# hcherkaoui/pybold

Measured on AMD Instinct MI355X. Metric: voxel-iterations/sec, higher is better.
Workload: dtype f16x2-split operands (22 bit), f32 accumulate, f64 iterate

## Files before the change

### include/pybold_hip.h

```cpp
#ifndef PYBOLD_HIP_H
#define PYBOLD_HIP_H

#include <stdint.h>

#ifdef __cplusplus
extern "C" {
#endif

#define PB_OK 0
#define PB_ERR_INVALID (-1)
#define PB_ERR_HIP (-2)

#define PB_FLAG_FORCE_GENERIC 1u
#define PB_FLAG_FORCE_FAST 2u
#define PB_FLAG_NO_PAIR 4u
#define PB_FLAG_FORCE_PAIR 8u
#define PB_FLAG_FORCE_WIDE 16u
#define PB_FLAG_DIRECT_FIR 64u
#define PB_FLAG_ONE_STREAM 128u
#define PB_FLAG_COLD_START 256u
#define PB_FLAG_NO_CERT 512u
#define PB_FLAG_CERT_NO_RESOLVE 2048u
#define PB_FLAG_FORCE_MFMA 16384u
#define PB_FLAG_NO_RHO_GUARD 32768u
// ... 18 lines not shown

int pb_fista_has_fast_path(int N, int K);

int pb_fista_which_kernel(int N, int K, int P, int with_cost_trace, int stop_mode, int wind);

int pb_fista_plan(int N, int K, int P, int stop_mode, int wind, int* n_main, int* main_form,
                  int* tail_form);
int pb_fista_plan_ex(int N, int K, int P, int stop_mode, int wind, unsigned flags, int* n_main,
                     int* main_form, int* tail_form);

int pb_fista_solve(const float* y_dev, int64_t ldy, int y_rep,
                   double* w_dev, int64_t ldw, int P, int N,
                   const double* taps_host, const double* taps_dev, int K,
                   double step, double lbda, const double* lbda_dev,
                   const double* betas_dev, int n_iter,
                   float* J_dev, int64_t ldj,
                   int stop_mode, double tol, int wind, int32_t* n_done_dev,
                   unsigned flags, void* stream);

int64_t pb_fista_work_len(int P, int y_rep);
#define PB_CAND_COUNT 10
int pb_fista_list_plan(int kind, int n, int n_max, int has_pair, int has_wide, int one_stream, int has_mfma2,
                       int beside_chunks, int32_t* ranges, int32_t* bounds);
int pb_fista_solve_ex(const float* y_dev, int64_t ldy, int y_rep,
                      double* w_dev, int64_t ldw, int P, int N,
                      const double* taps_host, const double* taps_dev, int K,
                      double step, double lbda, const double* lbda_dev,
                      const double* betas_dev, int n_iter,
                      float* J_dev, int64_t ldj,
                      int stop_mode, double tol, int wind, int32_t* n_done_dev,
                      unsigned flags, void* stream,
                      const double* lmax_dev, double dense_ratio, int32_t* work_dev, int64_t work_len);

#define PB_PATH_DENSE_RATIO 0.19
#define PB_PATH_DENSE_RATIO_LONG 0.22
#define PB_PATH_DENSE_RATIO_LONGER 0.26
int64_t pb_fista_path_work_len(int P);
int pb_fista_solve_path(const float* y_dev, int64_t ldy, int y_rep, double* w_dev, int64_t ldw, int P, int N,
                        const double* taps_host, const double* taps_dev, int K, double step,
                        const double* lbda_dev, const double* lmax_dev, double dense_ratio,
                        const double* betas_dev, int n_iter, int32_t* n_done_dev, int32_t* work_dev,
                        int64_t work_len, unsigned flags, void* stream);

int pb_fista_outputs(const double* w_dev, int64_t ldw, int P, int N,
                     const double* taps_dev, int K,
                     double* z_dev, int64_t ldz, double* x_dev, int64_t ldx,
// ... 138 lines not shown
```

### pybold_amd/_lib.py

```python
import ctypes
import os

_HERE = os.path.dirname(os.path.abspath(__file__))
LIB_PATH = os.environ.get("PYBOLD_HIP_LIB") or os.path.join(_HERE, "libpybold_hip.so")

PB_FLAG_FORCE_GENERIC = 1
PB_FLAG_FORCE_FAST = 2
PB_FLAG_NO_PAIR = 4
PB_FLAG_FORCE_PAIR = 8
PB_FLAG_FORCE_WIDE = 16
PB_FLAG_ONE_LAUNCH = 32
PB_FLAG_DIRECT_FIR = 64
PB_FLAG_ONE_STREAM = 128
PB_FLAG_COLD_START = 256
PB_FLAG_NO_CERT = 512
PB_FLAG_FORCE_CERT = 1024
PB_FLAG_CERT_NO_RESOLVE = 2048
PB_FLAG_NO_PARTITION = 4096
PB_FLAG_NO_MFMA = 8192
PB_FLAG_FORCE_MFMA = 16384
PB_FLAG_NO_RHO_GUARD = 32768
PB_FLAG_FORCE_MFMA2 = 65536
PB_FLAG_ONLY_DENSE = 131072
PB_FLAG_ONLY_SPARSE = 262144
# ... 7 lines not shown
_c_i64 = ctypes.c_int64
_c_dbl = ctypes.c_double
_ptr = ctypes.c_void_p

SIGNATURES = {
    "pb_version": (_c_int, []),
    "pb_init": (_c_int, []),
    "pb_last_error": (ctypes.c_char_p, []),
    "pb_fista_has_fast_path": (_c_int, [_c_int, _c_int]),
    "pb_fista_which_kernel": (_c_int, [_c_int, _c_int, _c_int, _c_int, _c_int, _c_int]),
    "pb_fista_plan": (_c_int, [_c_int, _c_int, _c_int, _c_int, _c_int, _ptr, _ptr, _ptr]),
    "pb_fista_plan_ex": (_c_int, [_c_int, _c_int, _c_int, _c_int, _c_int, ctypes.c_uint, _ptr, _ptr, _ptr]),
    "pb_fista_solve": (_c_int, [
        _ptr, _c_i64, _c_int,
        _ptr, _c_i64, _c_int, _c_int,
        _ptr, _ptr, _c_int,
        _c_dbl, _c_dbl, _ptr,
        _ptr, _c_int,
        _ptr, _c_i64,
        _c_int, _c_dbl, _c_int, _ptr,
        ctypes.c_uint, _ptr]),
    "pb_fista_work_len": (_c_i64, [_c_int, _c_int]),
    "pb_fista_list_plan": (_c_int, [_c_int, _c_int, _c_int, _c_int, _c_int, _c_int, _c_int, _c_int, _ptr, _ptr]),
    "pb_fista_solve_ex": (_c_int, [
        _ptr, _c_i64, _c_int,
        _ptr, _c_i64, _c_int, _c_int,
        _ptr, _ptr, _c_int,
        _c_dbl, _c_dbl, _ptr,
        _ptr, _c_int,
        _ptr, _c_i64,
        _c_int, _c_dbl, _c_int, _ptr,
        ctypes.c_uint, _ptr,
        _ptr, _c_dbl, _ptr, _c_i64]),
    "pb_fista_solve_backtrack_d": (_c_int, [
        _ptr, _c_i64, _c_int, _ptr, _c_i64, _c_int, _c_int,
        _ptr, _c_int, _c_dbl, _c_dbl, _c_int,
        _c_dbl, _ptr, _ptr, _c_int,
        _ptr, _ptr, _ptr, ctypes.c_uint, _ptr]),
    "pb_fista_path_work_len": (_c_i64, [_c_int]),
    "pb_fista_solve_path": (_c_int, [
        _ptr, _c_i64, _c_int,
        _ptr, _c_i64, _c_int, _c_int,
        _ptr, _ptr, _c_int,
        _c_dbl, _ptr, _ptr, _c_dbl,
        _ptr, _c_int,
        _ptr, _ptr, _c_i64,
# ... 133 lines not shown
```

### pybold_amd/csrc/capi.hip

```cpp
#include "../../include/pybold_hip.h"

#include <cstdarg>
#include <cstdlib>
#include <cstdio>
#include <cmath>
#include <cstring>
#include <map>
#include <mutex>

#include "fista_fast.h"
#include "generic.h"
#include "launch_fast.h"
#include "fista_pair.h"
#include "fista_pair_ffa.h"
#include "fista_exact.h"
#include "fista_exact_split.h"
#include "fista_auto.h"
#include "fista_exact_pp.h"
#include "blind.h"
#include "fista_mfma.h"
#include "fista_mfma2.h"
#include "fista_mfma4.h"
#include "path.h"
#include "dispatch.h"
// ... 35 lines not shown
  const int64_t rounds = ((int64_t)V + AUTO_SPLIT_RESIDENT_WGS - 1) / AUTO_SPLIT_RESIDENT_WGS;
  const int64_t per = (int64_t)(nb_sub_iter > 0 ? nb_sub_iter : 1) * (rounds > 0 ? rounds : 1);
  const int64_t c = AUTO_SPLIT_LAUNCH_ITERS / per;
  return (int)(c < 1 ? 1 : c);
}

constexpr int MAD_DAUB_NMAX = 8192;
template <typename TY>
int mad_daub_impl(const TY* y_dev, int64_t ldy, int V, int N, double c, double* sigma_dev, void* stream, const char* name) {
  if (V < 0 || ldy < N) return fail(PB_ERR_INVALID, "%s: bad size", name);
  if (N < 5 || N > MAD_DAUB_NMAX) return fail(PB_ERR_INVALID, "%s: N=%d outside 5..%d scans", name, N, MAD_DAUB_NMAX);
  if (!(c > 0.0)) return fail(PB_ERR_INVALID, "%s: c must be positive", name);
  if (V == 0) return PB_OK;
  if (!y_dev || !sigma_dev) return fail(PB_ERR_INVALID, "%s: NULL pointer", name);
  int n2 = 1;
  while (n2 < (N + 5) / 2) n2 <<= 1;
  hipLaunchKernelGGL((pb::mad_daub_kernel<TY>), dim3(V), dim3(pb::GEN_THREADS), (size_t)n2 * sizeof(double), (hipStream_t)stream,
                     y_dev, ldy, N, c, n2, sigma_dev);
  return check_launch(name);
}
struct SideStream {
  hipStream_t stream = nullptr;
  hipEvent_t fork = nullptr, join = nullptr;
  bool ok = false;
};
std::mutex g_side_mutex;

SideStream* side_stream_locked() {
  static std::map<int, SideStream> per_dev;
  int dev = 0;
  if (hipGetDevice(&dev) != hipSuccess) return nullptr;
  SideStream& ss = per_dev[dev];
  if (!ss.ok && ss.stream == nullptr) {
    int least = 0, greatest = 0;
    if (hipDeviceGetStreamPriorityRange(&least, &greatest) != hipSuccess) { least = greatest = 0; (void)hipGetLastError(); }
    if (hipStreamCreateWithPriority(&ss.stream, hipStreamNonBlocking, greatest) == hipSuccess &&
        hipEventCreateWithFlags(&ss.fork, hipEventDisableTiming) == hipSuccess &&
        hipEventCreateWithFlags(&ss.join, hipEventDisableTiming) == hipSuccess)
      ss.ok = true;
    else
      (void)hipGetLastError();
  }
  return ss.ok ? &ss : nullptr;
}

bool stream_is_capturing(hipStream_t st) {
  hipStreamCaptureStatus cs = hipStreamCaptureStatusNone;
  if (hipStreamIsCapturing(st, &cs) != hipSuccess) {
    (void)hipGetLastError();
    return true;
  }
  return cs != hipStreamCaptureStatusNone;
}
struct WorkLayout { int64_t ranges, lmax, total; };
WorkLayout work_layout(int P, int V) {
  const int64_t nblk = ((int64_t)P + pb::PATH_PER_BLOCK - 1) / pb::PATH_PER_BLOCK;
  WorkLayout w;
  w.ranges = ((int64_t)P + 2 + 2 * nblk + 8 + 1) & ~(int64_t)1;
  w.lmax = w.ranges + 3 * 2 * pb::CAND_COUNT + 4;
  w.total = w.lmax + 2 * (int64_t)V + 8;
  return w;
}
int32_t* own_workspace(void* stream, int64_t need, int64_t* len) {
  static std::mutex mu;
  static std::map<std::pair<int, void*>, std::pair<int32_t*, int64_t>> cache;
  int dev = 0;
  if (hipGetDevice(&dev) != hipSuccess) { (void)hipGetLastError(); return nullptr; }
  std::lock_guard<std::mutex> lock(mu);
  auto& e = cache[std::make_pair(dev, stream)];
  if (e.second < need) {
    int32_t* fresh = nullptr;
    const int64_t want = need + need / 4;
    if (hipMalloc((void**)&fresh, (size_t)want * sizeof(int32_t)) != hipSuccess) { (void)hipGetLastError(); return nullptr; }
    e.first = fresh;
    e.second = want;
  }
  *len = e.second;
  return e.first;
}

template <int KIND>
int launch_op(const double* x, int64_t ldx, double* out, int64_t ldo, int V, int n_src, int n_dst,
              const double* taps, int K, void* stream, const char* name) {
// ... 187 lines not shown
template <class LF>
int launch(const LF& lf, int form, const pb::FistaArgs& b, hipStream_t st, bool exact_rule = false) {
  static const char* const kernel[] = {"fista_generic_kernel", "fista_fast_kernel", "fista_pair_ffa_kernel", "fista_fast_kernel(wide)",
                                       "fista_mfma_kernel", "fista_mfma2_kernel / fista_mfma4_kernel"};
  if (lf(form, b, st, exact_rule) != 0) return fail(PB_ERR_INVALID, "%s: the kernel of form %d rejected its launch", lf.name, form);
  return check_launch(kernel[form]);
}

struct Side {
  std::unique_lock<std::mutex> lock{g_side_mutex, std::defer_lock};
  SideStream* ss = nullptr;
  bool forked = false;
  void take() {
    lock.lock();
    ss = side_stream_locked();
  }
  int fork(hipStream_t user, const char* name) {
    if (forked) return PB_OK;
    if (hipEventRecord(ss->fork, user) != hipSuccess || hipStreamWaitEvent(ss->stream, ss->fork, 0) != hipSuccess)
      return fail(PB_ERR_HIP, "%s: fork to the side stream failed", name);
    forked = true;
    return PB_OK;
  }
  int join(hipStream_t user, const char* name) {
    if (!forked) return PB_OK;
    forked = false;
    if (hipEventRecord(ss->join, ss->stream) != hipSuccess || hipStreamWaitEvent(user, ss->join, 0) != hipSuccess)
      return fail(PB_ERR_HIP, "%s: join of the side stream failed", name);
    return PB_OK;
  }
};

template <class LF>
int run_passes(const pb::FistaArgs& a, int base, int main_form, int rest_form, bool resolve, const LF& lf, hipStream_t st) {
  pb::FistaArgs b = a;
  if (base > 0) {
    b.P = base;
    const int rc = launch(lf, main_form, b, st);
    if (rc != PB_OK) return rc;
  }
  if (base < a.P) {
    b = a;
    b.p0 = base;
    const int rc = launch(lf, rest_form, b, st);
    if (rc != PB_OK) return rc;
  }
// ... 64 lines not shown
    s.dense.pass_mult = 2;
    s.dense.rem_num16 = MFMA4_MIN_R_NUM;
  }
  s.dense.backup_form = s.sparse.backup_form = s.flagged.backup_form = r.backup_wide ? FORM_WIDE : FORM_FAST1;
  s.sparse.min_pair = SPLIT_MIN_P;
  return s;
}
bool list_has_form(const Route& r, int form, int list) {
  const bool lng = r.path == PATH_PART_LONG;
  if (form == FORM_MFMA) return list <= 1 && r.mfma != nullptr;
  if (form == FORM_MFMA2) return list <= 1 && (lng || r.has_mfma2);
  if (list == 1) return false;
  if (form == FORM_PAIR) return list != 3 && r.has_pair;
  if (form == FORM_WIDE) return lng ? r.backup_wide : r.has_wide;
  return !lng || !r.backup_wide;
}
int cand_bound(const Route& r, int c, int P) {
  if (r.path == PATH_PART_SHORT) return pb::cand_max_slots(c, P, wave_slots());
  return (c == pb::CAND_MFMA2 || c == pb::CAND_PAIR0 || c == pb::CAND_FAST0 || c == pb::CAND_WIDE) ? P : 0;
}

template <class LF>
int solve_list(const Route& r, const pb::FistaArgs& a, const LF& lf, hipStream_t user, Side& side, const int32_t* work_dev,
               const int32_t* ranges, int list, bool exact_rule) {
  pb::FistaArgs b = a;
  b.perm = work_dev;
  b.n_dense = work_dev + a.P;
  b.perm_side = list == 3 ? 3 : 1;
  int rc = PB_OK;
  for (int c = 0; c < pb::CAND_COUNT && rc == PB_OK; ++c) {
    const int form = pb::cand_form(c);
    if (!list_has_form(r, form, list) || (pb::cand_side(c) && !side.ss)) continue;
    if ((c == pb::CAND_PAIR1 || c == pb::CAND_FAST1) && !side.ss) continue;
    b.grid_slots = cand_bound(r, c, a.P);
    if (b.grid_slots <= 0) continue;
    if (c >= pb::CAND_FIRST_AFTER_FORK && side.ss) rc = side.fork(user, lf.name);
    if (rc != PB_OK) break;
    b.range = ranges + 2 * c;
    rc = launch(lf, form, b, (pb::cand_side(c) && side.ss) ? side.ss->stream : user, exact_rule);
  }
  const int rj = side.join(user, lf.name);
  return rj != PB_OK ? rj : rc;
}

void launch_lmax_pass(const pb::FistaArgs& a, int V_series, const double* taps_host, double* lm, double gamma_f64, double gamma_vec,
                      hipStream_t st) {
  const int N = a.N, K = a.K;
  pb::LmaxTaps lt;
  double run = 0.0, csum = 0.0;
  for (int k = 0; k < pb::LMAX_KT; ++k) lt.h[k] = k < K ? (float)taps_host[k] : 0.0f;
  for (int t = 0; t < N; ++t) { if (t < K) run += taps_host[t]; csum += std::fabs(run); }
  const double unit = csum / std::sqrt((double)N);
  const float f64_bound = gamma_f64 > 0.0 ? (float)(gamma_f64 * unit) : 0.0f, vec_bound = gamma_vec > 0.0 ? (float)(gamma_vec * unit) : 0.0f;
  const dim3 grid((unsigned)((V_series + 3) / 4)), block(256);
  if (N <= 320) hipLaunchKernelGGL((pb::lmax_wave_kernel<5>), grid, block, 4 * (64 * 5 + pb::LMAX_KT) * sizeof(float), st, a.y, a.ldy, V_series, N, lt, K, lm, f64_bound, vec_bound);
  else if (N <= 640) hipLaunchKernelGGL((pb::lmax_wave_kernel<10>), grid, block, 4 * (64 * 10 + pb::LMAX_KT) * sizeof(float), st, a.y, a.ldy, V_series, N, lt, K, lm, f64_bound, vec_bound);
  else hipLaunchKernelGGL((pb::lmax_wave_kernel<21>), grid, block, 4 * (64 * 21 + pb::LMAX_KT) * sizeof(float), st, a.y, a.ldy, V_series, N, lt, K, lm, f64_bound, vec_bound);
}

int launch_partition(const pb::ClassPred& cp, int P, int32_t* work_dev, const pb::PlanSpec& front, const pb::PlanSpec& back,
                     int32_t* rg_front, int32_t* rg_back, int32_t* rg_ill, const char* what, hipStream_t st) {
  const int nblk = (P + pb::PATH_PER_BLOCK - 1) / pb::PATH_PER_BLOCK;
  hipLaunchKernelGGL(pb::path_count_kernel, dim3(nblk), dim3(pb::PATH_THREADS), 0, st, cp, P, work_dev);
  hipLaunchKernelGGL(pb::path_scan_kernel, dim3(1), dim3(pb::PATH_THREADS), 0, st, P, nblk, work_dev, front, back, rg_front, rg_back, rg_ill);
  hipLaunchKernelGGL(pb::path_scatter_kernel, dim3(nblk), dim3(pb::PATH_THREADS), 0, st, cp, P, work_dev);
  return check_launch(what);
}

void launch_generic(const pb::FistaArgs& a, const double* taps_dev, int K, int wind, bool with_j, bool f64, int grid, hipStream_t st) {
  void (*const kernel)(pb::FistaArgs, const double*, int, int) =
      !f64 ? (with_j ? pb::fista_generic_kernel<true> : pb::fista_generic_kernel<false>)
           : (with_j ? pb::fista_generic_kernel<true, true> : pb::fista_generic_kernel<false, true>);
  hipLaunchKernelGGL(kernel, dim3(grid), dim3(pb::GEN_THREADS), (size_t)gen_lds_doubles(a.N, K, a.stop_mode, wind) * sizeof(double), st,
                     a, taps_dev, K, wind);
}

template <class LF>
int run_partition(const Route& r, const pb::FistaArgs& a, const LF& lf, hipStream_t user, const double* taps_host,
                  const double* taps_dev, unsigned flags, double dense_ratio, int32_t* work_dev) {
  const int P = a.P, N = a.N, K = a.K, V_series = (P + a.y_rep - 1) / a.y_rep;
  const bool one_stream = r.path == PATH_PART_LONG || (flags & PB_FLAG_ONE_STREAM) != 0 || stream_is_capturing(user);
  const PartitionSpecs sp = partition_specs(r, N, one_stream);
  const WorkLayout wl = work_layout(P, V_series);
  const ExactEntry* ill_exact = pick_exact_any(N, K, a.stop_mode, a.wind, nullptr);
  const bool ill_generic = !ill_exact && taps_dev && gen_lds_doubles(N, K, a.stop_mode, a.wind) <= LDS_DOUBLES_MAX;
  const bool guard = !(flags & PB_FLAG_NO_ILL_GUARD);
  double* lmax = reinterpret_cast<double*>(work_dev + wl.lmax);
  launch_lmax_pass(a, V_series, taps_host, lmax, (guard && (ill_exact || ill_generic)) ? PART_GAMMA_F64 : 0.0,
                   guard ? part_gamma_matrix_pipe(N, K) : 0.0, user);
  int32_t* rg_dense = work_dev + wl.ranges;
  int32_t* rg_sparse = rg_dense + 2 * pb::CAND_COUNT;
  int32_t* rg_flag = rg_sparse + 2 * pb::CAND_COUNT;
  int32_t* rg_ill = rg_flag + 2 * pb::CAND_COUNT;
  const double ratio = (r.path == PATH_PART_SHORT && !r.mfma) ? 0.0
                       : dense_ratio > 0.0 ? dense_ratio
                       : N > 640 ? PB_PATH_DENSE_RATIO_LONGER : (N > MFMA1_NMAX ? PB_PATH_DENSE_RATIO_LONG : PB_PATH_DENSE_RATIO);
  pb::PlanSpec front = sp.dense;
  front.merged = 1;
  int rc = launch_partition(pb::ClassPred{a.lbda_vec, a.lbda, lmax, a.y_rep, ratio, nullptr}, P, work_dev, front, sp.sparse, rg_dense,
                            rg_sparse, rg_ill, "partition", user);
  if (rc != PB_OK) return rc;
  Side side;
  if (!one_stream) side.take();
  const bool only_dense = (flags & PB_FLAG_ONLY_DENSE) != 0, only_sparse = (flags & PB_FLAG_ONLY_SPARSE) != 0;
  rc = solve_list(r, a, lf, user, side, work_dev, rg_dense, only_dense ? 1 : (only_sparse ? 2 : 0), false);
  if (rc != PB_OK || only_dense || only_sparse) return rc;
  if (ill_exact || ill_generic) {
    pb::FistaArgs b = a;
    b.perm = work_dev;
    b.perm_side = 1;
    b.range = rg_ill;
    if (ill_exact) {
      b.grid_slots = P;
      if (ill_exact->fn(b, taps_host, K, a.J != nullptr, a.stop_mode, user) != 0)
        return fail(PB_ERR_INVALID, "%s: float64 kernel rejected the launch (ill-conditioned series)", lf.name);
    } else {
      launch_generic(b, taps_dev, K, a.wind, a.J != nullptr, false, P < 2048 ? P : 2048, user);
    }
    rc = check_launch("float64 kernel (ill-conditioned series)");
    if (rc != PB_OK) return rc;
  }
  const pb::PlanSpec none{0, 0, 0, 0, 1, 0, 0, sp.dense.slots};
  rc = launch_partition(pb::ClassPred{nullptr, 0.0, nullptr, 1, 0.0, a.n_done}, P, work_dev, sp.flagged, none, rg_flag, nullptr, nullptr,
                        "partition(handed back)", user);
  if (rc != PB_OK) return rc;
  side.ss = nullptr;
  return solve_list(r, a, lf, user, side, work_dev, rg_flag, 3, true);
}

int outputs_impl(const double* w_dev, int64_t ldw, int P, int N, const double* taps_dev, int64_t ldt, int K, double* z_dev,
                 int64_t ldz, double* x_dev, int64_t ldx, void* stream, bool pp, const char* name) {
  if (P < 0 || N < 1 || K < 1 || ldw < N || (pp && ldt < K) || (z_dev && ldz < N) || (x_dev && ldx < N))
    return fail(PB_ERR_INVALID, "%s: bad size", name);
  if (2 * (int64_t)N + K + 8 > LDS_DOUBLES_MAX) return fail(PB_ERR_INVALID, "%s: N=%d K=%d exceeds LDS", name, N, K);
  if (P == 0 || (!z_dev && !x_dev)) return PB_OK;
  if (!w_dev || !taps_dev) return fail(PB_ERR_INVALID, "%s: NULL pointer", name);
  const size_t lds = (size_t)(2 * N + K + 8) * sizeof(double);
  hipLaunchKernelGGL(pb::outputs_kernel, dim3(P), dim3(pb::GEN_THREADS), lds, (hipStream_t)stream,
                     w_dev, ldw, N, taps_dev, ldt, K, z_dev, ldz, x_dev, ldx);
  return check_launch(name);
}

pb::HrfModel hrf_model(double a_peak, double loc_peak, double a_under, double loc_under, double ratio) {
  return pb::HrfModel{a_peak, loc_peak, lgamma(a_peak), a_under, loc_under, lgamma(a_under), ratio,
                      pb::hrf_int_power(a_peak), pb::hrf_int_power(a_under), std::exp(-lgamma(a_peak)),
                      std::exp(-lgamma(a_under))};
}

pb::FistaArgs fista_args(int P, int N, int K, int n_iter, int y_rep, int64_t ldy, double* w, int64_t ldw, double step,
                         double lbda, const double* lbda_vec, const double* betas, int stop_mode, double tol,
// ... 102 lines not shown
  if (gen_lds_doubles(N, K, stop_mode, wind) > LDS_DOUBLES_MAX)
    return fail(PB_ERR_INVALID, "pb_fista_solve: N=%d K=%d wind=%d exceeds LDS", N, K, wind);
  launch_generic(a, taps_dev, K, wind, J_dev != nullptr, false, P, user);
  return check_launch("fista_generic_kernel");
}

int pb_fista_list_plan(int kind, int n, int n_max, int has_pair, int has_wide, int one_stream, int has_mfma2,
                       int beside_chunks, int32_t* ranges, int32_t* bounds) {
  if (kind < 1 || kind > 3 || n < 0 || n_max < n) return fail(PB_ERR_INVALID, "pb_fista_list_plan: bad argument");
  Piece pc[pb::MAX_PIECES];
  int npc = 0;
  const double slots = wave_slots();
  if (n > 0 && kind == 1) npc = pb::plan_pieces_mfma(n, has_pair != 0, has_wide != 0, false, one_stream != 0, has_mfma2 != 0, beside_chunks, slots, pc);
  else if (n > 0 && kind == 2) npc = pb::plan_pieces(n, has_pair != 0, has_wide != 0, false, one_stream != 0, slots, pc);
  else if (kind == 3 && n_max > 0)
    npc = pb::plan_partitioned(n, n_max, has_pair != 0, has_wide != 0, one_stream != 0, has_mfma2 != 0, beside_chunks, slots, pc);
  int32_t rg[2 * pb::CAND_COUNT];
  const int rc = pb::plan_to_candidates(pc, npc, rg);
  for (int c = 0; c < pb::CAND_COUNT; ++c) {
    if (ranges) { ranges[2 * c] = rg[2 * c]; ranges[2 * c + 1] = rg[2 * c + 1]; }
    if (bounds) bounds[c] = pb::cand_max_slots(c, n_max, slots);
  }
  if (rc != 0) return fail(PB_ERR_INVALID, "pb_fista_list_plan: a piece of the plan found its candidate launch taken (n=%d)", n);
  g_err[0] = 0;
  return PB_OK;
}

int64_t pb_fista_work_len(int P, int y_rep) {
  if (P < 0 || y_rep < 1) return 0;
  return work_layout(P, (P + y_rep - 1) / y_rep).total;
}

int pb_fista_solve_ex(const float* y_dev, int64_t ldy, int y_rep, double* w_dev, int64_t ldw, int P,
                      int N, const double* taps_host, const double* taps_dev, int K, double step,
                      double lbda, const double* lbda_dev, const double* betas_dev, int n_iter, float* J_dev,
                      int64_t ldj, int stop_mode, double tol, int wind, int32_t* n_done_dev,
                      unsigned flags, void* stream, const double* lmax_dev, double dense_ratio,
                      int32_t* work_dev, int64_t work_len) {
  return solve_impl(y_dev, ldy, y_rep, w_dev, ldw, P, N, taps_host, taps_dev, K, step, lbda, lbda_dev, betas_dev, n_iter,
                    J_dev, ldj, stop_mode, tol, wind, n_done_dev, flags, stream, lmax_dev, dense_ratio, work_dev, work_len);
}

int pb_fista_solve(const float* y_dev, int64_t ldy, int y_rep, double* w_dev, int64_t ldw, int P,
                   int N, const double* taps_host, const double* taps_dev, int K, double step,
                   double lbda,
                   const double* lbda_dev, const double* betas_dev, int n_iter, float* J_dev,
// ... 530 lines not shown
```

### pybold_amd/csrc/path.h

```cpp
#pragma once
#include <hip/hip_runtime.h>
#include <stdint.h>

#include "plan.h"

namespace pb {

constexpr int PATH_THREADS = 256, PATH_PER_THREAD = 16, PATH_PER_BLOCK = PATH_THREADS * PATH_PER_THREAD;

struct ClassPred {
  const double* lbda;
  double lbda_s;
  const double* lmax;
  int y_rep;
  double ratio;
  const int32_t* n_done;
};

__device__ __forceinline__ int path_class(const ClassPred& c, int p) {
  if (c.n_done) return c.n_done[p] < 0 ? 0 : 1;
  const double lm = c.lmax[p / c.y_rep];
  if (lm < 0.0) return 2;
  const double lb = c.lbda ? c.lbda[p] : c.lbda_s;
  return lb < c.ratio * lm ? 0 : 1;
}

__host__ __device__ inline int path_nill_offset(int nblk) { return 1 + 2 * nblk; }

__global__ __launch_bounds__(PATH_THREADS) void path_count_kernel(ClassPred cp, int P, int32_t* work) {
  __shared__ int part[2][PATH_THREADS / 64];
  const int p0 = blockIdx.x * PATH_PER_BLOCK + threadIdx.x * PATH_PER_THREAD;
  int c = 0, ci = 0;
  for (int i = 0; i < PATH_PER_THREAD; ++i) {
    if (p0 + i >= P) break;
    const int k = path_class(cp, p0 + i);
    c += k == 0;
    ci += k == 2;
  }
  for (int o = 32; o > 0; o >>= 1) { c += __shfl_xor(c, o, 64); ci += __shfl_xor(ci, o, 64); }
  if ((threadIdx.x & 63) == 0) { part[0][threadIdx.x >> 6] = c; part[1][threadIdx.x >> 6] = ci; }
  __syncthreads();
  if (threadIdx.x == 0) {
    work[P + 1 + blockIdx.x] = part[0][0] + part[0][1] + part[0][2] + part[0][3];
    work[P + 1 + gridDim.x + blockIdx.x] = part[1][0] + part[1][1] + part[1][2] + part[1][3];
  }
}

struct PlanSpec {
  int kind;
  int has_pair, has_wide, one_launch, one_stream, has_mfma2, beside_chunks;
  double slots;
  int backup_form = FORM_WIDE;
  int min_pair = 1024;
  int pass_mult = 4;
  int rem_num16 = 5;
  int merged = 0;
};
__device__ __forceinline__ void plan_list(const PlanSpec& sp, int n, int32_t* ranges);
__device__ __forceinline__ void plan_call(const PlanSpec& front, const PlanSpec& back, int n_d, int P, int32_t* ranges);

__global__ __launch_bounds__(PATH_THREADS) void path_scan_kernel(int P, int nblk, int32_t* work, PlanSpec front, PlanSpec back,
                                                                  int32_t* ranges_front, int32_t* ranges_back, int32_t* range_ill) {
  __shared__ int buf[PATH_THREADS];
  __shared__ int carry;
  int total[2] = {0, 0};
  for (int which = 0; which < 2; ++which) {
    if (threadIdx.x == 0) carry = 0;
    __syncthreads();
    int32_t* cnt = work + P + 1 + which * nblk;
    for (int b0 = 0; b0 < nblk; b0 += PATH_THREADS) {
      const int b = b0 + (int)threadIdx.x;
      const int v = b < nblk ? cnt[b] : 0;
      buf[threadIdx.x] = v;
      __syncthreads();
      for (int o = 1; o < PATH_THREADS; o <<= 1) {
        const int add = threadIdx.x >= (unsigned)o ? buf[threadIdx.x - o] : 0;
        __syncthreads();
        buf[threadIdx.x] += add;
        __syncthreads();
      }
      if (b < nblk) cnt[b] = carry + buf[threadIdx.x] - v;
      __syncthreads();
      if (threadIdx.x == PATH_THREADS - 1) carry += buf[PATH_THREADS - 1];
      __syncthreads();
    }
    total[which] = carry;
    __syncthreads();
  }
  if (threadIdx.x == 0) {
    const int n_front = total[0], n_ill = total[1], P_eff = P - n_ill;
    work[P] = n_front;
    work[P + path_nill_offset(nblk)] = n_ill;
    if (range_ill) { range_ill[0] = P_eff; range_ill[1] = P; }
    if (ranges_front && front.merged) plan_call(front, back, n_front, P_eff, ranges_front);
    else {
      if (ranges_front) plan_list(front, n_front, ranges_front);
      if (ranges_back) plan_list(back, P_eff - n_front, ranges_back);
    }
  }
}

__global__ __launch_bounds__(PATH_THREADS) void path_scatter_kernel(ClassPred cp, int P, int32_t* work) {
  __shared__ int buf[2][PATH_THREADS];
  const int p0 = blockIdx.x * PATH_PER_BLOCK + threadIdx.x * PATH_PER_THREAD;
  unsigned mask = 0, maski = 0;
  int c = 0, ci = 0;
  for (int i = 0; i < PATH_PER_THREAD; ++i) {
    if (p0 + i >= P) break;
    const int k = path_class(cp, p0 + i);
    if (k == 0) { mask |= 1u << i; ++c; }
    if (k == 2) { maski |= 1u << i; ++ci; }
  }
  buf[0][threadIdx.x] = c;
  buf[1][threadIdx.x] = ci;
  __syncthreads();
  for (int o = 1; o < PATH_THREADS; o <<= 1) {
    const int add = threadIdx.x >= (unsigned)o ? buf[0][threadIdx.x - o] : 0;
    const int addi = threadIdx.x >= (unsigned)o ? buf[1][threadIdx.x - o] : 0;
    __syncthreads();
    buf[0][threadIdx.x] += add;
    buf[1][threadIdx.x] += addi;
    __syncthreads();
  }
  const int n_front = work[P];
  int d = work[P + 1 + blockIdx.x] + buf[0][threadIdx.x] - c;
  int e = work[P + 1 + gridDim.x + blockIdx.x] + buf[1][threadIdx.x] - ci;
  for (int i = 0; i < PATH_PER_THREAD; ++i) {
    const int p = p0 + i;
    if (p >= P) break;
    if (mask & (1u << i)) work[d++] = p;
    else if (maski & (1u << i)) work[P - 1 - (e++)] = p;
    else work[n_front + (p - d - e)] = p;
  }
}

__device__ __forceinline__ void plan_list(const PlanSpec& sp, int n, int32_t* ranges) {
  Piece pc[MAX_PIECES];
  int npc = 0;
  if (n > 0 && sp.kind == 1)
    npc = plan_pieces_mfma(n, sp.has_pair != 0, sp.has_wide != 0, sp.one_launch != 0, sp.one_stream != 0, sp.has_mfma2 != 0,
                           sp.beside_chunks, sp.slots, pc);
  else if (n > 0 && sp.kind == 2)
    npc = plan_pieces(n, sp.has_pair != 0, sp.has_wide != 0, sp.one_launch != 0, sp.one_stream != 0, sp.slots, pc);
  else if (n > 0 && sp.kind == 3) {
    const int pass = (int)sp.slots * sp.pass_mult;
    int base = (n / pass) * pass;
    if (sp.one_launch || n - base > pass * sp.rem_num16 / 16) base = n;
    if (base > 0) pc[npc++] = Piece{FORM_MFMA2, 0, base, false, false};
    if (base < n) pc[npc++] = Piece{sp.backup_form, base, n, false, false};
  } else if (n > 0 && sp.kind == 4) {
    pc[npc++] = Piece{(sp.has_pair && n >= sp.min_pair) ? FORM_PAIR : sp.backup_form, 0, n, false, false};
  }
  if (plan_to_candidates(pc, npc, ranges) != 0) {
    for (int c = 0; c < 2 * CAND_COUNT; ++c) ranges[c] = 0;
    const int c = sp.kind == 1 ? CAND_MFMA : (sp.kind == 3 ? CAND_MFMA2 : ((sp.kind == 4 && sp.backup_form == FORM_WIDE) ? CAND_WIDE : CAND_FAST0));
    ranges[2 * c + 1] = n;
  }
}

__device__ __forceinline__ void plan_call(const PlanSpec& front, const PlanSpec& back, int n_d, int P, int32_t* ranges) {
  Piece pc[MAX_PIECES];
  int npc = 0;
  if (front.kind == 1) {
    npc = plan_partitioned(n_d, P, front.has_pair != 0, front.has_wide != 0, front.one_stream != 0, front.has_mfma2 != 0,
                           front.beside_chunks, front.slots, pc);
  } else {
    const int pass = (int)front.slots * front.pass_mult;
    int base = (n_d / pass) * pass;
    if (n_d - base > pass * front.rem_num16 / 16) base = n_d;
    if (base > 0) pc[npc++] = Piece{FORM_MFMA2, 0, base, false, false};
    if (base < P) pc[npc++] = Piece{(back.has_pair && P - base >= back.min_pair) ? FORM_PAIR : back.backup_form, base, P, false, false};
  }
  if (plan_to_candidates(pc, npc, ranges) != 0) {
    for (int c = 0; c < 2 * CAND_COUNT; ++c) ranges[c] = 0;
    const int c = (front.kind != 1 && back.backup_form == FORM_WIDE) ? CAND_WIDE : CAND_FAST0;
    ranges[2 * c + 1] = P;
  }
}

constexpr int LMAX_KT = 64;
struct LmaxTaps { float h[LMAX_KT]; };

template <int SL>
__global__ __launch_bounds__(256) void lmax_wave_kernel(const float* y, int64_t ldy, int V, int N, LmaxTaps tp, int K, double* out,
                                                        float f64_bound, float vec_bound) {
  extern __shared__ float lm_smem[];
  const int lane = threadIdx.x & 63, wv = threadIdx.x >> 6;
  const int v = blockIdx.x * 4 + wv;
  if (v >= V) return;
  float* s = lm_smem + wv * (64 * SL + LMAX_KT);
  const float* yrow = y + (int64_t)v * ldy;
  float loc[SL];
  float run = 0.0f, ysq = 0.0f;
#pragma unroll
  for (int j = SL - 1; j >= 0; --j) {
    const int t = lane * SL + j;
    const float yv = t < N ? yrow[t] : 0.0f;
    ysq = fmaf(yv, yv, ysq);
    run += yv;
    loc[j] = run;
  }
  float above = run;
#pragma unroll
  for (int o = 1; o < 64; o <<= 1) {
    const float t = __shfl_down(above, o, 64);
    above += (lane + o < 64) ? t : 0.0f;
  }
  above -= run;
#pragma unroll
// ... 28 lines not shown
```

Before: 4.651 billion.

## Overlap ill-conditioned and handed-back solves on side stream; fuse partition scan into count

The separate single-block scan kernel is removed. The count kernel now finishes the plan itself in its last block, found with an atomic ticket, and the scatter kernel computes its own prefix sums by summing the earlier blocks' counts. The float64 solve for ill-conditioned series is forked early onto the side stream. The handed-back partition and solve are chained after the matrix launches on the side stream and only rescan the matrix ranges, writing into a second work list. This is meant to cut launch count and serial dependencies between stages, at the cost of ticket resets, extra workspace and more complex stream and event ordering.

New measurement: 4.674 billion (median of 6 runs). Within noise of the previous version (+0.5%).

```diff
diff --git a/include/pybold_hip.h b/include/pybold_hip.h
--- a/include/pybold_hip.h
+++ b/include/pybold_hip.h
@@ -64,6 +64,8 @@
 #define PB_CAND_COUNT 10
 int pb_fista_list_plan(int kind, int n, int n_max, int has_pair, int has_wide, int one_stream, int has_mfma2,
                        int beside_chunks, int32_t* ranges, int32_t* bounds);
+int pb_fista_partition_plan(int handed_back, int n_front, int n_ill, int P, int has_pair, int has_wide, int one_stream,
+                            int has_mfma2, int beside_chunks, int32_t* ranges_front, int32_t* ranges_back, int32_t* range_ill);
 int pb_fista_solve_ex(const float* y_dev, int64_t ldy, int y_rep,
                       double* w_dev, int64_t ldw, int P, int N,
                       const double* taps_host, const double* taps_dev, int K,
diff --git a/pybold_amd/_lib.py b/pybold_amd/_lib.py
--- a/pybold_amd/_lib.py
+++ b/pybold_amd/_lib.py
@@ -53,6 +53,7 @@
         ctypes.c_uint, _ptr]),
     "pb_fista_work_len": (_c_i64, [_c_int, _c_int]),
     "pb_fista_list_plan": (_c_int, [_c_int, _c_int, _c_int, _c_int, _c_int, _c_int, _c_int, _c_int, _ptr, _ptr]),
+    "pb_fista_partition_plan": (_c_int, [_c_int, _c_int, _c_int, _c_int, _c_int, _c_int, _c_int, _c_int, _c_int, _ptr, _ptr, _ptr]),
     "pb_fista_solve_ex": (_c_int, [
         _ptr, _c_i64, _c_int,
         _ptr, _c_i64, _c_int, _c_int,
diff --git a/pybold_amd/csrc/capi.hip b/pybold_amd/csrc/capi.hip
--- a/pybold_amd/csrc/capi.hip
+++ b/pybold_amd/csrc/capi.hip
@@ -81,6 +81,7 @@
 struct SideStream {
   hipStream_t stream = nullptr;
   hipEvent_t fork = nullptr, join = nullptr;
+  hipEvent_t early = nullptr, chain = nullptr;
   bool ok = false;
 };
 std::mutex g_side_mutex;
@@ -95,7 +96,9 @@
     if (hipDeviceGetStreamPriorityRange(&least, &greatest) != hipSuccess) { least = greatest = 0; (void)hipGetLastError(); }
     if (hipStreamCreateWithPriority(&ss.stream, hipStreamNonBlocking, greatest) == hipSuccess &&
         hipEventCreateWithFlags(&ss.fork, hipEventDisableTiming) == hipSuccess &&
-        hipEventCreateWithFlags(&ss.join, hipEventDisableTiming) == hipSuccess)
+        hipEventCreateWithFlags(&ss.join, hipEventDisableTiming) == hipSuccess &&
+        hipEventCreateWithFlags(&ss.early, hipEventDisableTiming) == hipSuccess &&
+        hipEventCreateWithFlags(&ss.chain, hipEventDisableTiming) == hipSuccess)
       ss.ok = true;
     else
       (void)hipGetLastError();
@@ -111,13 +114,14 @@
   }
   return cs != hipStreamCaptureStatusNone;
 }
-struct WorkLayout { int64_t ranges, lmax, total; };
+struct WorkLayout { int64_t ranges, lmax, list2, total; };
 WorkLayout work_layout(int P, int V) {
   const int64_t nblk = ((int64_t)P + pb::PATH_PER_BLOCK - 1) / pb::PATH_PER_BLOCK;
   WorkLayout w;
   w.ranges = ((int64_t)P + 2 + 2 * nblk + 8 + 1) & ~(int64_t)1;
   w.lmax = w.ranges + 3 * 2 * pb::CAND_COUNT + 4;
-  w.total = w.lmax + 2 * (int64_t)V + 8;
+  w.list2 = w.lmax + 2 * (int64_t)V + 8;
+  w.total = w.list2 + (int64_t)P + 2 + 2 * nblk + 8;
   return w;
 }
 int32_t* own_workspace(void* stream, int64_t need, int64_t* len) {
@@ -351,6 +355,12 @@
     forked = true;
     return PB_OK;
   }
+  int fork_at(hipEvent_t ev, hipStream_t user, const char* name) {
+    if (hipEventRecord(ev, user) != hipSuccess || hipStreamWaitEvent(ss->stream, ev, 0) != hipSuccess)
+      return fail(PB_ERR_HIP, "%s: fork to the side stream failed", name);
+    forked = true;
+    return PB_OK;
+  }
   int join(hipStream_t user, const char* name) {
     if (!forked) return PB_OK;
     forked = false;
@@ -461,29 +471,37 @@
 
 template <class LF>
 int solve_list(const Route& r, const pb::FistaArgs& a, const LF& lf, hipStream_t user, Side& side, const int32_t* work_dev,
-               const int32_t* ranges, int list, bool exact_rule) {
+               const int32_t* ranges, int list, bool exact_rule, hipEvent_t after_matrix = nullptr) {
   pb::FistaArgs b = a;
   b.perm = work_dev;
   b.n_dense = work_dev + a.P;
   b.perm_side = list == 3 ? 3 : 1;
+  const auto queued = [&](int c) {
+    if (!list_has_form(r, pb::cand_form(c), list) || (pb::cand_side(c) && !side.ss)) return false;
+    if ((c == pb::CAND_PAIR1 || c == pb::CAND_FAST1) && !side.ss) return false;
+    return cand_bound(r, c, a.P) > 0;
+  };
+  const int last_matrix = queued(pb::CAND_MFMA2) ? pb::CAND_MFMA2 : (queued(pb::CAND_MFMA) ? pb::CAND_MFMA : -1);
   int rc = PB_OK;
+  if (after_matrix && last_matrix < 0 && hipEventRecord(after_matrix, user) != hipSuccess)
+    rc = fail(PB_ERR_HIP, "%s: fork to the side stream failed", lf.name);
   for (int c = 0; c < pb::CAND_COUNT && rc == PB_OK; ++c) {
-    const int form = pb::cand_form(c);
-    if (!list_has_form(r, form, list) || (pb::cand_side(c) && !side.ss)) continue;
-    if ((c == pb::CAND_PAIR1 || c == pb::CAND_FAST1) && !side.ss) continue;
+    if (!queued(c)) continue;
     b.grid_slots = cand_bound(r, c, a.P);
-    if (b.grid_slots <= 0) continue;
     if (c >= pb::CAND_FIRST_AFTER_FORK && side.ss) rc = side.fork(user, lf.name);
     if (rc != PB_OK) break;
     b.range = ranges + 2 * c;
-    rc = launch(lf, form, b, (pb::cand_side(c) && side.ss) ? side.ss->stream : user, exact_rule);
-  }
+    rc = launch(lf, pb::cand_form(c), b, (pb::cand_side(c) && side.ss) ? side.ss->stream : user, exact_rule);
+    if (rc == PB_OK && after_matrix && c == last_matrix && hipEventRecord(after_matrix, user) != hipSuccess)
+      rc = fail(PB_ERR_HIP, "%s: fork to the side stream failed", lf.name);
+  }
+  if (after_matrix) return rc;
   const int rj = side.join(user, lf.name);
   return rj != PB_OK ? rj : rc;
 }
 
 void launch_lmax_pass(const pb::FistaArgs& a, int V_series, const double* taps_host, double* lm, double gamma_f64, double gamma_vec,
-                      hipStream_t st) {
+                      int32_t* tickets, hipStream_t st) {
   const int N = a.N, K = a.K;
   pb::LmaxTaps lt;
   double run = 0.0, csum = 0.0;
@@ -492,16 +510,16 @@
   const double unit = csum / std::sqrt((double)N);
   const float f64_bound = gamma_f64 > 0.0 ? (float)(gamma_f64 * unit) : 0.0f, vec_bound = gamma_vec > 0.0 ? (float)(gamma_vec * unit) : 0.0f;
   const dim3 grid((unsigned)((V_series + 3) / 4)), block(256);
-  if (N <= 320) hipLaunchKernelGGL((pb::lmax_wave_kernel<5>), grid, block, 4 * (64 * 5 + pb::LMAX_KT) * sizeof(float), st, a.y, a.ldy, V_series, N, lt, K, lm, f64_bound, vec_bound);
-  else if (N <= 640) hipLaunchKernelGGL((pb::lmax_wave_kernel<10>), grid, block, 4 * (64 * 10 + pb::LMAX_KT) * sizeof(float), st, a.y, a.ldy, V_series, N, lt, K, lm, f64_bound, vec_bound);
-  else hipLaunchKernelGGL((pb::lmax_wave_kernel<21>), grid, block, 4 * (64 * 21 + pb::LMAX_KT) * sizeof(float), st, a.y, a.ldy, V_series, N, lt, K, lm, f64_bound, vec_bound);
+  if (N <= 320) hipLaunchKernelGGL((pb::lmax_wave_kernel<5>), grid, block, 4 * (64 * 5 + pb::LMAX_KT) * sizeof(float), st, a.y, a.ldy, V_series, N, lt, K, lm, f64_bound, vec_bound, tickets);
+  else if (N <= 640) hipLaunchKernelGGL((pb::lmax_wave_kernel<10>), grid, block, 4 * (64 * 10 + pb::LMAX_KT) * sizeof(float), st, a.y, a.ldy, V_series, N, lt, K, lm, f64_bound, vec_bound, tickets);
+  else hipLaunchKernelGGL((pb::lmax_wave_kernel<21>), grid, block, 4 * (64 * 21 + pb::LMAX_KT) * sizeof(float), st, a.y, a.ldy, V_series, N, lt, K, lm, f64_bound, vec_bound, tickets);
 }
 
 int launch_partition(const pb::ClassPred& cp, int P, int32_t* work_dev, const pb::PlanSpec& front, const pb::PlanSpec& back,
-                     int32_t* rg_front, int32_t* rg_back, int32_t* rg_ill, const char* what, hipStream_t st) {
+                     int32_t* rg_front, int32_t* rg_back, int32_t* rg_ill, int32_t* ticket, const char* what, hipStream_t st) {
   const int nblk = (P + pb::PATH_PER_BLOCK - 1) / pb::PATH_PER_BLOCK;
-  hipLaunchKernelGGL(pb::path_count_kernel, dim3(nblk), dim3(pb::PATH_THREADS), 0, st, cp, P, work_dev);
-  hipLaunchKernelGGL(pb::path_scan_kernel, dim3(1), dim3(pb::PATH_THREADS), 0, st, P, nblk, work_dev, front, back, rg_front, rg_back, rg_ill);
+  hipLaunchKernelGGL(pb::path_count_kernel, dim3(nblk), dim3(pb::PATH_THREADS), 0, st, cp, P, work_dev, front, back,
+                     pb::PlanOut{rg_front, rg_back, rg_ill, ticket});
   hipLaunchKernelGGL(pb::path_scatter_kernel, dim3(nblk), dim3(pb::PATH_THREADS), 0, st, cp, P, work_dev);
   return check_launch(what);
 }
@@ -525,46 +543,74 @@
   const bool ill_generic = !ill_exact && taps_dev && gen_lds_doubles(N, K, a.stop_mode, a.wind) <= LDS_DOUBLES_MAX;
   const bool guard = !(flags & PB_FLAG_NO_ILL_GUARD);
   double* lmax = reinterpret_cast<double*>(work_dev + wl.lmax);
-  launch_lmax_pass(a, V_series, taps_host, lmax, (guard && (ill_exact || ill_generic)) ? PART_GAMMA_F64 : 0.0,
-                   guard ? part_gamma_matrix_pipe(N, K) : 0.0, user);
   int32_t* rg_dense = work_dev + wl.ranges;
   int32_t* rg_sparse = rg_dense + 2 * pb::CAND_COUNT;
   int32_t* rg_flag = rg_sparse + 2 * pb::CAND_COUNT;
   int32_t* rg_ill = rg_flag + 2 * pb::CAND_COUNT;
+  int32_t* tickets = rg_ill + 2;
+  int32_t* work2 = work_dev + wl.list2;
+  launch_lmax_pass(a, V_series, taps_host, lmax, (guard && (ill_exact || ill_generic)) ? PART_GAMMA_F64 : 0.0,
+                   guard ? part_gamma_matrix_pipe(N, K) : 0.0, tickets, user);
   const double ratio = (r.path == PATH_PART_SHORT && !r.mfma) ? 0.0
                        : dense_ratio > 0.0 ? dense_ratio
                        : N > 640 ? PB_PATH_DENSE_RATIO_LONGER : (N > MFMA1_NMAX ? PB_PATH_DENSE_RATIO_LONG : PB_PATH_DENSE_RATIO);
   pb::PlanSpec front = sp.dense;
   front.merged = 1;
   int rc = launch_partition(pb::ClassPred{a.lbda_vec, a.lbda, lmax, a.y_rep, ratio, nullptr}, P, work_dev, front, sp.sparse, rg_dense,
-                            rg_sparse, rg_ill, "partition", user);
+                            rg_sparse, rg_ill, tickets, "partition", user);
   if (rc != PB_OK) return rc;
+  const bool only_dense = (flags & PB_FLAG_ONLY_DENSE) != 0, only_sparse = (flags & PB_FLAG_ONLY_SPARSE) != 0;
+  const bool whole = !only_dense && !only_sparse;
   Side side;
   if (!one_stream) side.take();
-  const bool only_dense = (flags & PB_FLAG_ONLY_DENSE) != 0, only_sparse = (flags & PB_FLAG_ONLY_SPARSE) != 0;
-  rc = solve_list(r, a, lf, user, side, work_dev, rg_dense, only_dense ? 1 : (only_sparse ? 2 : 0), false);
-  if (rc != PB_OK || only_dense || only_sparse) return rc;
-  if (ill_exact || ill_generic) {
+  const bool beside = side.ss != nullptr && whole, chain_beside = beside && !r.cert;
+  const hipStream_t side_st = side.ss ? side.ss->stream : user;
+  const auto finish = [&](int rc_) {
+    const int rj = side.join(user, lf.name);
+    return rj != PB_OK ? rj : rc_;
+  };
+  const auto solve_ill = [&](hipStream_t st) {
+    if (!ill_exact && !ill_generic) return (int)PB_OK;
     pb::FistaArgs b = a;
     b.perm = work_dev;
     b.perm_side = 1;
     b.range = rg_ill;
     if (ill_exact) {
       b.grid_slots = P;
-      if (ill_exact->fn(b, taps_host, K, a.J != nullptr, a.stop_mode, user) != 0)
+      if (ill_exact->fn(b, taps_host, K, a.J != nullptr, a.stop_mode, st) != 0)
         return fail(PB_ERR_INVALID, "%s: float64 kernel rejected the launch (ill-conditioned series)", lf.name);
     } else {
-      launch_generic(b, taps_dev, K, a.wind, a.J != nullptr, false, P < 2048 ? P : 2048, user);
+      launch_generic(b, taps_dev, K, a.wind, a.J != nullptr, false, P < 2048 ? P : 2048, st);
     }
-    rc = check_launch("float64 kernel (ill-conditioned series)");
-    if (rc != PB_OK) return rc;
+    return check_launch("float64 kernel (ill-conditioned series)");
+  };
+  if (beside && (ill_exact || ill_generic)) {
+    rc = side.fork_at(side.ss->early, user, lf.name);
+    if (rc == PB_OK) rc = solve_ill(side_st);
+    if (rc != PB_OK) return finish(rc);
+  }
+  rc = solve_list(r, a, lf, user, side, work_dev, rg_dense, only_dense ? 1 : (only_sparse ? 2 : 0), false,
+                  chain_beside ? side.ss->chain : nullptr);
+  if (rc != PB_OK || !whole) return finish(rc);
+  if (!beside) {
+    rc = solve_ill(user);
+    if (rc != PB_OK) return finish(rc);
+  }
+  hipStream_t chain_st = user;
+  if (chain_beside) {
+    if (hipStreamWaitEvent(side_st, side.ss->chain, 0) != hipSuccess)
+      return finish(fail(PB_ERR_HIP, "%s: fork to the side stream failed", lf.name));
+    side.forked = true;
+    chain_st = side_st;
   }
   const pb::PlanSpec none{0, 0, 0, 0, 1, 0, 0, sp.dense.slots};
-  rc = launch_partition(pb::ClassPred{nullptr, 0.0, nullptr, 1, 0.0, a.n_done}, P, work_dev, sp.flagged, none, rg_flag, nullptr, nullptr,
-                        "partition(handed back)", user);
-  if (rc != PB_OK) return rc;
-  side.ss = nullptr;
-  return solve_list(r, a, lf, user, side, work_dev, rg_flag, 3, true);
+  pb::ClassPred handed{nullptr, 0.0, nullptr, 1, 0.0, a.n_done};
+  if (!r.cert) { handed.src_list = work_dev; handed.src_ranges = rg_dense; }
+  rc = launch_partition(handed, P, work2, sp.flagged, none, rg_flag, nullptr, nullptr, tickets + 1, "partition(handed back)", chain_st);
+  if (rc != PB_OK) return finish(rc);
+  Side one;
+  rc = solve_list(r, a, lf, chain_st, one, work2, rg_flag, 3, true);
+  return finish(rc);
 }
 
 int outputs_impl(const double* w_dev, int64_t ldw, int P, int N, const double* taps_dev, int64_t ldt, int K, double* z_dev,
@@ -713,6 +759,23 @@
     if (bounds) bounds[c] = pb::cand_max_slots(c, n_max, slots);
   }
   if (rc != 0) return fail(PB_ERR_INVALID, "pb_fista_list_plan: a piece of the plan found its candidate launch taken (n=%d)", n);
+  g_err[0] = 0;
+  return PB_OK;
+}
+
+int pb_fista_partition_plan(int handed_back, int n_front, int n_ill, int P, int has_pair, int has_wide, int one_stream,
+                            int has_mfma2, int beside_chunks, int32_t* ranges_front, int32_t* ranges_back, int32_t* range_ill) {
+  if (n_front < 0 || n_ill < 0 || P < 0 || (int64_t)n_front + n_ill > P || !ranges_front)
+    return fail(PB_ERR_INVALID, "pb_fista_partition_plan: bad argument");
+  const double slots = wave_slots();
+  const int pair = has_pair != 0, wide = has_wide != 0, os = one_stream != 0;
+  pb::PlanSpec front{1, pair, wide, 0, os, has_mfma2 != 0, beside_chunks, slots}, back{2, pair, wide, 0, os, 0, 0, slots};
+  front.merged = 1;
+  if (handed_back) {
+    front = pb::PlanSpec{2, 0, wide, 0, 1, 0, 0, slots};
+    back = pb::PlanSpec{0, 0, 0, 0, 1, 0, 0, slots};
+  }
+  pb::plan_lists(front, back, n_front, n_ill, P, ranges_front, handed_back ? nullptr : ranges_back, range_ill);
   g_err[0] = 0;
   return PB_OK;
 }
diff --git a/pybold_amd/csrc/path.h b/pybold_amd/csrc/path.h
--- a/pybold_amd/csrc/path.h
+++ b/pybold_amd/csrc/path.h
@@ -15,10 +15,19 @@
   int y_rep;
   double ratio;
   const int32_t* n_done;
+  const int32_t* src_list = nullptr;
+  const int32_t* src_ranges = nullptr;
 };
 
 __device__ __forceinline__ int path_class(const ClassPred& c, int p) {
-  if (c.n_done) return c.n_done[p] < 0 ? 0 : 1;
+  if (c.n_done) {
+    if (c.src_list) {
+      const int32_t* r = c.src_ranges;
+      if (!((p >= r[2 * CAND_MFMA] && p < r[2 * CAND_MFMA + 1]) || (p >= r[2 * CAND_MFMA2] && p < r[2 * CAND_MFMA2 + 1]))) return 1;
+      p = c.src_list[p];
+    }
+    return c.n_done[p] < 0 ? 0 : 1;
+  }
   const double lm = c.lmax[p / c.y_rep];
   if (lm < 0.0) return 2;
   const double lb = c.lbda ? c.lbda[p] : c.lbda_s;
@@ -27,23 +36,13 @@
 
 __host__ __device__ inline int path_nill_offset(int nblk) { return 1 + 2 * nblk; }
 
-__global__ __launch_bounds__(PATH_THREADS) void path_count_kernel(ClassPred cp, int P, int32_t* work) {
-  __shared__ int part[2][PATH_THREADS / 64];
-  const int p0 = blockIdx.x * PATH_PER_BLOCK + threadIdx.x * PATH_PER_THREAD;
-  int c = 0, ci = 0;
-  for (int i = 0; i < PATH_PER_THREAD; ++i) {
-    if (p0 + i >= P) break;
-    const int k = path_class(cp, p0 + i);
-    c += k == 0;
-    ci += k == 2;
-  }
+__device__ __forceinline__ void path_block_sum2(int& c, int& ci, int (*part)[PATH_THREADS / 64]) {
   for (int o = 32; o > 0; o >>= 1) { c += __shfl_xor(c, o, 64); ci += __shfl_xor(ci, o, 64); }
   if ((threadIdx.x & 63) == 0) { part[0][threadIdx.x >> 6] = c; part[1][threadIdx.x >> 6] = ci; }
   __syncthreads();
-  if (threadIdx.x == 0) {
-    work[P + 1 + blockIdx.x] = part[0][0] + part[0][1] + part[0][2] + part[0][3];
-    work[P + 1 + gridDim.x + blockIdx.x] = part[1][0] + part[1][1] + part[1][2] + part[1][3];
-  }
+  c = part[0][0] + part[0][1] + part[0][2] + part[0][3];
+  ci = part[1][0] + part[1][1] + part[1][2] + part[1][3];
+  __syncthreads();
 }
 
 struct PlanSpec {
@@ -56,53 +55,71 @@
   int rem_num16 = 5;
   int merged = 0;
 };
-__device__ __forceinline__ void plan_list(const PlanSpec& sp, int n, int32_t* ranges);
-__device__ __forceinline__ void plan_call(const PlanSpec& front, const PlanSpec& back, int n_d, int P, int32_t* ranges);
-
-__global__ __launch_bounds__(PATH_THREADS) void path_scan_kernel(int P, int nblk, int32_t* work, PlanSpec front, PlanSpec back,
-                                                                  int32_t* ranges_front, int32_t* ranges_back, int32_t* range_ill) {
-  __shared__ int buf[PATH_THREADS];
-  __shared__ int carry;
-  int total[2] = {0, 0};
-  for (int which = 0; which < 2; ++which) {
-    if (threadIdx.x == 0) carry = 0;
-    __syncthreads();
-    int32_t* cnt = work + P + 1 + which * nblk;
-    for (int b0 = 0; b0 < nblk; b0 += PATH_THREADS) {
-      const int b = b0 + (int)threadIdx.x;
-      const int v = b < nblk ? cnt[b] : 0;
-      buf[threadIdx.x] = v;
-      __syncthreads();
-      for (int o = 1; o < PATH_THREADS; o <<= 1) {
-        const int add = threadIdx.x >= (unsigned)o ? buf[threadIdx.x - o] : 0;
-        __syncthreads();
-        buf[threadIdx.x] += add;
-        __syncthreads();
-      }
-      if (b < nblk) cnt[b] = carry + buf[threadIdx.x] - v;
-      __syncthreads();
-      if (threadIdx.x == PATH_THREADS - 1) carry += buf[PATH_THREADS - 1];
-      __syncthreads();
-    }
-    total[which] = carry;
-    __syncthreads();
-  }
+struct PlanOut {
+  int32_t* front;
+  int32_t* back;
+  int32_t* ill;
+  int32_t* ticket;
+};
+PB_HD void plan_list(const PlanSpec& sp, int n, int32_t* ranges);
+PB_HD void plan_call(const PlanSpec& front, const PlanSpec& back, int n_d, int P, int32_t* ranges);
+
+PB_HD void plan_lists(const PlanSpec& front, const PlanSpec& back, int n_front, int n_ill, int P, int32_t* rg_front, int32_t* rg_back,
+                      int32_t* rg_ill) {
+  const int P_eff = P - n_ill;
+  if (rg_ill) { rg_ill[0] = P_eff; rg_ill[1] = P; }
+  if (rg_front && front.merged) plan_call(front, back, n_front, P_eff, rg_front);
+  else {
+    if (rg_front) plan_list(front, n_front, rg_front);
+    if (rg_back) plan_list(back, P_eff - n_front, rg_back);
+  }
+}
+
+__global__ __launch_bounds__(PATH_THREADS) void path_count_kernel(ClassPred cp, int P, int32_t* work, PlanSpec front, PlanSpec back,
+                                                                   PlanOut out) {
+  __shared__ int part[2][PATH_THREADS / 64];
+  __shared__ int last;
+  const int nblk = (int)gridDim.x;
+  const int p0 = blockIdx.x * PATH_PER_BLOCK + threadIdx.x * PATH_PER_THREAD;
+  int c = 0, ci = 0;
+  for (int i = 0; i < PATH_PER_THREAD; ++i) {
+    if (p0 + i >= P) break;
+    const int k = path_class(cp, p0 + i);
+    c += k == 0;
+    ci += k == 2;
+  }
+  path_block_sum2(c, ci, part);
   if (threadIdx.x == 0) {
-    const int n_front = total[0], n_ill = total[1], P_eff = P - n_ill;
-    work[P] = n_front;
-    work[P + path_nill_offset(nblk)] = n_ill;
-    if (range_ill) { range_ill[0] = P_eff; range_ill[1] = P; }
-    if (ranges_front && front.merged) plan_call(front, back, n_front, P_eff, ranges_front);
-    else {
-      if (ranges_front) plan_list(front, n_front, ranges_front);
-      if (ranges_back) plan_list(back, P_eff - n_front, ranges_back);
-    }
+    work[P + 1 + blockIdx.x] = c;
+    work[P + 1 + nblk + blockIdx.x] = ci;
+    __threadfence();
+    last = atomicAdd(out.ticket, 1) == nblk - 1;
+  }
+  __syncthreads();
+  if (!last) return;
+  __threadfence();
+  c = ci = 0;
+  for (int b = threadIdx.x; b < nblk; b += PATH_THREADS) {
+    c += __hip_atomic_load(work + P + 1 + b, __ATOMIC_RELAXED, __HIP_MEMORY_SCOPE_AGENT);
+    ci += __hip_atomic_load(work + P + 1 + nblk + b, __ATOMIC_RELAXED, __HIP_MEMORY_SCOPE_AGENT);
+  }
+  path_block_sum2(c, ci, part);
+  if (threadIdx.x == 0) {
+    work[P] = c;
+    work[P + path_nill_offset(nblk)] = ci;
+    plan_lists(front, back, c, ci, P, out.front, out.back, out.ill);
+    *out.ticket = 0;
   }
 }
 
 __global__ __launch_bounds__(PATH_THREADS) void path_scatter_kernel(ClassPred cp, int P, int32_t* work) {
   __shared__ int buf[2][PATH_THREADS];
+  __shared__ int part[2][PATH_THREADS / 64];
+  const int nblk = (int)gridDim.x;
   const int p0 = blockIdx.x * PATH_PER_BLOCK + threadIdx.x * PATH_PER_THREAD;
+  int before = 0, beforei = 0;
+  for (int b = threadIdx.x; b < (int)blockIdx.x; b += PATH_THREADS) { before += work[P + 1 + b]; beforei += work[P + 1 + nblk + b]; }
+  path_block_sum2(before, beforei, part);
   unsigned mask = 0, maski = 0;
   int c = 0, ci = 0;
   for (int i = 0; i < PATH_PER_THREAD; ++i) {
@@ -123,18 +140,18 @@
     __syncthreads();
   }
   const int n_front = work[P];
-  int d = work[P + 1 + blockIdx.x] + buf[0][threadIdx.x] - c;
-  int e = work[P + 1 + gridDim.x + blockIdx.x] + buf[1][threadIdx.x] - ci;
+  int d = before + buf[0][threadIdx.x] - c;
+  int e = beforei + buf[1][threadIdx.x] - ci;
   for (int i = 0; i < PATH_PER_THREAD; ++i) {
     const int p = p0 + i;
     if (p >= P) break;
-    if (mask & (1u << i)) work[d++] = p;
+    if (mask & (1u << i)) work[d++] = cp.src_list ? cp.src_list[p] : p;
     else if (maski & (1u << i)) work[P - 1 - (e++)] = p;
-    else work[n_front + (p - d - e)] = p;
-  }
-}
-
-__device__ __forceinline__ void plan_list(const PlanSpec& sp, int n, int32_t* ranges) {
+    else if (!cp.n_done) work[n_front + (p - d - e)] = p;
+  }
+}
+
+PB_HD void plan_list(const PlanSpec& sp, int n, int32_t* ranges) {
   Piece pc[MAX_PIECES];
   int npc = 0;
   if (n > 0 && sp.kind == 1)
@@ -158,7 +175,7 @@
   }
 }
 
-__device__ __forceinline__ void plan_call(const PlanSpec& front, const PlanSpec& back, int n_d, int P, int32_t* ranges) {
+PB_HD void plan_call(const PlanSpec& front, const PlanSpec& back, int n_d, int P, int32_t* ranges) {
   Piece pc[MAX_PIECES];
   int npc = 0;
   if (front.kind == 1) {
@@ -183,8 +200,9 @@
 
 template <int SL>
 __global__ __launch_bounds__(256) void lmax_wave_kernel(const float* y, int64_t ldy, int V, int N, LmaxTaps tp, int K, double* out,
-                                                        float f64_bound, float vec_bound) {
+                                                        float f64_bound, float vec_bound, int32_t* tickets) {
   extern __shared__ float lm_smem[];
+  if (blockIdx.x == 0 && threadIdx.x == 0) { tickets[0] = 0; tickets[1] = 0; }
   const int lane = threadIdx.x & 63, wv = threadIdx.x >> 6;
   const int v = blockIdx.x * 4 + wv;
   if (v >= V) return;
```
